# whabacivch/GC-SLAM

Measured on AMD Instinct MI355X. Metric: scans/sec (14-step pipeline) at 64k pts/scan, higher is better.
Workload: dtype f64

## Files before the change

gc-slam_amd/csrc/gcs_capi.cpp:

```cpp
#include "gcslam_hip.h"

#include <hip/hip_runtime.h>
#include <math.h>
#include <rccl/rccl.h>
#include <string.h>

#include <algorithm>
#include <atomic>
#include <sys/syscall.h>
#include <unistd.h>
#include <chrono>
#include <condition_variable>
#include <mutex>
#include <thread>
#include <string>
#include <vector>

#include "gcs_atlas.h"
#include "gcs_host.h"
#include "gcs_imu_odom_core.h"
#include "gcs_kernels.h"
#include "gcs_layout.h"
#include "gcs_live.h"
#include "gcs_math.h"
// ... 107 lines not shown
    int nblk;
    gcs_pmap* pm;
    int32_t n12, ncl;
    int32_t tiles12[GCS_LIVE_MAX_TILES], clear12[GCS_LIVE_MAX_TILES];
    int64_t tids12[GCS_LIVE_MAX_TILES];
    double ts12;
    int64_t seq12, next12;
    gcs_pmap_update_config ucfg;
    gcs_pmap_update_inputs uin;
  };
  PushJob push_jobs[2]{};
  int push_rc = 0;
  std::string push_err;
  uint64_t* h_gate = nullptr;
  uint64_t* d_gate = nullptr;
  double* d_gate_xi = nullptr;
  uint64_t gate_seq = 0, gate_next = 0;
  bool gate_on = false;
  bool gate_withhold = false;
  bool device_preint = false;
  bool device_imu_odom = false;
  bool io_dev_pending = false;
  hipStream_t io_stream = nullptr;
  double* h_io_stage = nullptr;
  double* d_io_win = nullptr;
  double* d_io_out = nullptr;
  double* h_io_out = nullptr;
  double* dh_io_out = nullptr;
  uint64_t* d_io_seq = nullptr;
  uint64_t io_seq = 0;
  int64_t io_rereads = 0, io_syncs = 0;
  hipEvent_t ev_preint = nullptr;
  bool ev_preint_pending = false;
  bool preint_pending = false;
  bool preint_host_pending = false;
  double* h_preint_in = nullptr;
  int64_t preint_in_cap = 0;
  double* h_preint_out = nullptr;
  int pts_blocks = 0;
  bool pts_fold_pending = false;
  double* d_scalars = nullptr;
  double* h_scalars = nullptr;
  double* d_scalars_mirror = nullptr;
  uint64_t mirror_seq = 0;
  int64_t mirror_scans = 0, mirror_rereads = 0, mirror_syncs = 0;
  int mirror_torn = 0;
  uint32_t h_err[4] = {0u, 0u, 0u, 0u};
  uint32_t* d_err = nullptr;
  uint32_t* d_members = nullptr;
  int capb = 32, capb_eff = 32;
  bool direct_buckets = true;
  bool sorted_sticky = false;
  bool use_direct = false;
  uint32_t spin_limit = 1u << 22;
  int inject_scan_fail = 0;
  bool legacy_points = [] {
    const char* e = getenv("GCSLAM_POINTS");
    return e && strcmp(e, "legacy") == 0;
  }();
  double* h_payload = nullptr;
  double* dh_payload = nullptr;
  double* d_payload = nullptr;
  double* d_payload_in = nullptr;
  int combine_delay_us = 0;
  int sendbuf_mode = -1;
  void* comm_seen = nullptr;
  int comm_world = 1;
  double* h_psum = nullptr;
  double* dh_psum = nullptr;
  hipStream_t comm_stream = nullptr;
  uint64_t pay_seq = 0;
  uint64_t* d_pay_seq = nullptr;
  int64_t pay_rereads = 0, pay_syncs = 0;
  Belief belief{};
  int map_mode = GCS_MAP_OWN;
  double map_rec[GCS_MAP_REC_LEN] = {};
  double lead_rec[GCS_MAP_REC_LEN] = {};
  bool have_lead_rec = false;
  bool prev_fac_valid = false;
  host::SpdFactor prev_fac;
  double prev_cov[DZ * DZ];
  double iw_nu[7], iw_Psi[7 * 36], Q[DZ * DZ];
  double last_dPsi[7 * 36], last_dnu[7];
  double meas_nu[3], meas_Psi[3 * 9], meas_cert[2] = {0.0, 0.0};
  double last_meas_dPsi[3 * 9], last_meas_dnu[3];
  bool have_last = false;
  int last_n_sel = 0, last_stride = 1;
  int budget_blocks = 0;
  double host_sums[10] = {};
  int64_t host_n[2] = {0, 0};
  static constexpr int kHostHist = 4096;
  std::vector<float> host_hist = std::vector<float>((size_t)kHostHist * 6, 0.0f);
  std::atomic<int64_t> worker_tid{0};
  bool budget_pending = false;
  bool self_budget = [] {
    const char* e = getenv("GCSLAM_SELF_BUDGET");
    return !(e && atoi(e) == 0);
  }();
  bool budget_self = false, recs_deferred = false;
  double2* d_mass_rows = nullptr;
  std::vector<double> wimu, wint;
  host::ImuOdomOut io;
  double grav[3] = {0.0, 0.0, 0.0};
  uint32_t timing_mask = 0;
  static constexpr int kEvRing = 256;
  std::vector<hipEvent_t> ev[kStages];
// ... 238 lines not shown
  a.t0 = t0;
  a.t1 = t1;
  memcpy(a.xi, xi, 6 * sizeof(double));
  memcpy(a.origin, c->cfg.lidar_origin, 3 * sizeof(double));
  a.tau = c->cfg.tau;
  a.bin_dirs = c->d_bin_dirs;
  a.n_bins = c->B;
  a.knn = c->d_knn;
  a.k = c->K;
  a.pools = c->d_pools;
  a.pool_bound = c->d_pool_bound;
  a.bin_ref = c->d_bin_ref;
  a.pool_width = c->pool_width;
  a.grid = c->G;
  a.recs = c->d_recs;
  a.keys = c->d_keys;
  a.slots = c->d_slots;
  a.counts = c->d_counts;
  if (c->use_direct) {
    a.members = c->d_members;
    a.capb = c->capb_eff;
    a.flags = c->d_flags;
    a.tile_shift = c->tile_shift;
    a.overflow = c->d_err + 2;
  }
  a.budget_partials = c->budget_self ? nullptr : c->d_partials;
  a.budget_blocks = c->budget_self ? 0 : c->budget_blocks;
  a.mass_rows = c->budget_self ? c->d_mass_rows : nullptr;
  c->recs_deferred = c->budget_self && c->cfg.mode == GCS_MODE_SCALE && !deskew_only;
  a.scalars = c->d_scalars;
  a.p0_out = p0_out;
  a.w_out = w_out;
  a.w_budget_out = wb_out;
  a.nearest_out = c->d_nearest;
  a.iz_out = iz_out;
  a.t_out = t_out;
  if (c->gate_next) {
    HIPCHK(c, launch_gate(c->d_gate, c->gate_next, c->d_gate_xi, c->d_err + 3, s));
    a.xi_dev = c->d_gate_xi;
    c->gate_next = 0;
  } else if (c->preint_pending) {
    a.xi_dev = c->d_gate_xi;
    c->preint_pending = false;
  }
  c->iz_valid = false;
  const bool scale = c->cfg.mode == GCS_MODE_SCALE && !deskew_only;
  if (deskew_only) {
    a.n_bins = 0;
    a.nearest_out = nullptr;
    a.members = nullptr;
  }
  c->pts_blocks = points_blocks(c->cap, scale);
  c->pts_fold_pending = scale && fold_later;
  MirrorArgs mir{};
  if (to_host && !c->pts_fold_pending) {
    mir.mirror = c->d_scalars_mirror;
    mir.err = c->d_err;
    mir.seq = ++c->mirror_seq;
    mir.torn = c->mirror_torn;
  }
  HIPCHK(c, launch_points(a, scale, c->d_part_pts, c->pts_blocks, !c->pts_fold_pending, s, ev.e0, ev.e1,
                          c->legacy_points, mir));
  return GCS_OK;
}

BinKernelArgs bin_args(gcs_ctx* c) {
  BinKernelArgs b{};
  b.recs = c->d_recs;
  b.perm = c->d_perm;
  if (c->use_direct) {
    b.members = c->d_members;
    b.capb = c->capb_eff;
  }
  b.starts = c->d_starts;
  b.counts = c->d_counts;
  b.flags = c->d_flags;
  b.tile_dirty = c->d_tile_dirty;
  b.tile_order = c->d_tile_order;
  b.tile_work = c->d_tile_work;
  b.rknn_off = c->d_rknn_off;
  b.rknn = c->d_rknn;
  b.rknn_local = c->d_rknn_local;
  b.tile_src_off = c->d_tile_src_off;
  b.tile_src = c->d_tile_src;
  b.bin_dirs = c->d_bin_dirs;
  b.map = c->d_map;
  b.n_bins = c->B;
  b.cap = c->cap;
  b.tile_bins = c->tile_bins;
  memcpy(b.origin, c->cfg.lidar_origin, 3 * sizeof(double));
  b.tau = c->cfg.tau;
  b.scan = c->d_scan;
  b.scalars = c->d_scalars;
  if (c->pts_fold_pending) {
    b.pts_partials = c->d_part_pts;
    b.pts_blocks = c->pts_blocks;
  }
  if (c->recs_deferred) {
    b.mass_rows = c->d_mass_rows;
    b.mass_nrows = c->pts_blocks;
  }
  if (c->d_counts) {
    b.zero_after = c->d_counts + c->B;
    b.n_zero_after = c->n_counts_words - c->B;
  }
  return b;
}

int stage_bins(gcs_ctx* c) {
  hipStream_t s = c->stream;
  BinKernelArgs b = bin_args(c);
  if (c->cfg.mode == GCS_MODE_SCALE) {
    if (!c->use_direct) {
      StageEv ev = stage_ev(c, ST_SORT);
      BucketArgs ba{};
      ba.n_bins = c->B;
      ba.k = c->K;
      ba.counts = c->d_counts;
      ba.keys = c->d_keys;
      ba.slots = c->d_slots;
      ba.knn = c->d_knn;
      ba.starts = c->d_starts;
      ba.scan_status = c->d_counts + c->B + 2;
      ba.scan_ticket = c->d_tickets;
      ba.slot_idx = c->d_sorted;
// ... 2599 lines not shown
```

gc-slam_amd/csrc/gcs_kernels.h:

```cpp
#pragma once
#include <hip/hip_runtime.h>
#include <stddef.h>
#include <stdint.h>

#include "gcs_layout.h"

namespace gcs {


struct ParseArgs {
  const uint8_t* data;
  int n, point_step;
  int off_x, off_y, off_z, off_ring, ring_datatype, off_t, t_datatype;
  double header_stamp;
  double R[9], tb[3];
  double* points;
  double* t;
  double* w;
  uint8_t* ring;
  uint32_t* ns_flag;
};

struct BudgetArgs {
  const double* w;
// ... 37 lines not shown
  int k;
  const int* pools;
  const float* pool_bound;
  const int* bin_ref;
  int pool_width, grid;
  PointRec* recs;
  uint32_t* keys;
  uint32_t* slots;
  uint32_t* counts;
  uint32_t* members;
  int capb;
  uint8_t* flags;
  int tile_shift;
  uint32_t* overflow;
  const double* budget_partials;
  int budget_blocks;
  double2* mass_rows;
  double* scalars;
  double* p0_out;
  double* w_out;
  double* w_budget_out;
  int* nearest_out;
  double* iz_out;
  double* t_out;
  const double* xi_dev;
};
constexpr uint64_t kGateTimeoutTicks = 20000000ull;

struct BucketArgs {
  int n_bins, k;
  const uint32_t* counts;
  const uint32_t* keys;
  const uint32_t* slots;
  const int* knn;
  uint32_t* starts;
  uint32_t* scan_status;
  uint32_t* scan_ticket;
  uint32_t* slot_idx;
  uint32_t* perm;
  uint8_t* flags;
  int tile_shift;
  uint32_t* err;
  uint32_t spin_limit;
  int inject_scan_fail;
};

struct BinKernelArgs {
  const PointRec* recs;
  const uint32_t* perm;
  const uint32_t* members;
  int capb;
  const uint32_t* starts;
  const uint32_t* counts;
  const uint8_t* flags;
  uint8_t* tile_dirty;
  const int* rknn_off;
  const int* rknn;
  const uint16_t* rknn_local;
  const int* tile_src_off;
  const int* tile_src;
  const double* bin_dirs;
  const double* map;
  int n_bins, cap;
  int tile_bins;
  double origin[3];
  double tau;
  double* scan;
  double* scalars;
  const double* pts_partials;
  int pts_blocks;
  const double2* mass_rows;
  int mass_nrows;
  uint32_t* zero_after;
  int n_zero_after;
  const int* tile_order;
  uint32_t* tile_work;
};

struct PushArgs {
  double R[9];
  double t[3];
  double Stt[9];
  double F[9];
  double G[9];
  double gamma;
};

hipError_t launch_parse(const ParseArgs& a, hipStream_t s);
hipError_t launch_budget(const BudgetArgs& a, int nblk, hipStream_t s, hipEvent_t e0, hipEvent_t e1);
int points_blocks(long cap, bool scale);
int points_max_blocks();
struct PreintArgs {
  const double* imu;
  int m;
  int n_tail;
  double tail_stamp;
  double t0, t1, sigma;
  double rotvec[3], gb[3], ab[3], g[3];
  int rotation_only;
  double* xi_dev;
  double* host_out;
};
hipError_t launch_preint(const PreintArgs& a, hipStream_t s);
constexpr int kImuOdomMaxM = 1024;
constexpr int kImuOdomStatWords = 24;
enum ImuOdomSmall : int {
  kIoPose0 = 0, kIoPosePred = 6, kIoMuPrev = 12, kIoMuInc = 34, kIoGravity = 56, kIoSigmaG = 59, kIoSigmaA = 68,
  kIoOdomPose = 77, kIoOdomCov = 83, kIoOdomTwist = 119, kIoOdomTwistCov = 125, kIoSmallLen = 161
};
struct ImuOdomDevArgs {
  const double* win;
  int m;
  double t_last_scan, t_scan, dt_sec;
  double planar_z_ref, planar_z_sigma, planar_vz_sigma;
  double* out;
  double* host;
  uint64_t* dseq;
};
hipError_t launch_imu_odom(const ImuOdomDevArgs& a, hipStream_t s);
hipError_t launch_gate(const uint64_t* gate, uint64_t seq, double* xi_out, uint32_t* err, hipStream_t s);
hipError_t launch_payload_out(const double* src, double* host, int n, uint64_t* dseq, hipStream_t s);
hipError_t launch_delay(int us, hipStream_t s);
hipError_t launch_points(const PointKernelArgs& a, bool scale, double* partials, int nblk, bool fold, hipStream_t s,
                         hipEvent_t e0, hipEvent_t e1, bool legacy = false, const MirrorArgs& mir = MirrorArgs{});
int scan_tiles(int n_bins);
hipError_t launch_bucketing(const BucketArgs& b, int n, hipStream_t s, hipEvent_t e0, hipEvent_t e1);
int bins_tile_for(long cap, int n_bins);
int bins_scale_blocks(int n_bins, int tile_bins);
int partial_stride(int nv);
size_t partials_need(long nblocks, int nv);
int bins_max_tile_sources(int tile_bins);
int bins_max_tile_entries(int tile_bins);
int bins_partial_nv();
int push_blocks(int n_bins);
hipError_t launch_bins_scale(const BinKernelArgs& a, double* partials, hipStream_t s, hipEvent_t e0, hipEvent_t e1,
                             hipEvent_t f0, hipEvent_t f1);
hipError_t launch_dense(const BinKernelArgs& a, double* bin_partials, double* partials, hipStream_t s, hipEvent_t e0,
                        hipEvent_t e1);
hipError_t launch_mf(const double* scan, const double* map, int B, double* partials, int nblk, double* scalars,
                     hipStream_t s, hipEvent_t e0, hipEvent_t e1);
hipError_t launch_pt(const double* scan, const double* map, const double* derived, int B, double* partials, int nblk,
                     double* scalars, const MirrorArgs& mir, const uint8_t* act, const uint8_t* touched,
                     hipStream_t s, hipEvent_t e0, hipEvent_t e1, PtClear clr = PtClear{});
hipError_t launch_tile_order(const uint8_t* active, const uint32_t* work, int n, int* order, hipStream_t s);
hipError_t launch_tile_order_variant(const uint8_t* active, const uint32_t* work, int n, int* order, bool xcd,
                                     hipStream_t s);
hipError_t launch_pushforward(const double* scan, double* map, double* derived, int B, const PushArgs& pa,
                              double* partials, double* scalars, const uint8_t* act, uint8_t* touched, hipStream_t s,
                              hipEvent_t e0, hipEvent_t e1);
hipError_t launch_map_derive(const double* map, double* derived, int B, double* partials, double* scalars,
                             uint8_t* touched, hipStream_t s);

}
```

gc-slam_amd/csrc/gcs_kernels.hip:

```cpp
#include <hip/hip_runtime.h>


#include "gcs_kernels.h"

#include <hip/hip_ext.h>
#include <string.h>
#include "gcs_layout.h"
#include "gcs_math.h"

namespace gcs {

constexpr int kBlock = 256;
constexpr int kWaves = kBlock / 64;

template <int NV>
__device__ __forceinline__ void wave_sum(double (&v)[NV]) {
#pragma unroll
  for (int off = 32; off >= 1; off >>= 1) {
#pragma unroll
    for (int k = 0; k < NV; ++k) v[k] += __shfl_xor(v[k], off, 64);
  }
}

template <int NV>
// ... 369 lines not shown
      for (int k = 0; k < 4; ++k) {
        v[0] += brow[k].x;
        v[1] += brow[k].y;
      }
      block_sum<2>(v, lds);
      if (threadIdx.x == 0) {
        s_mass[0] = v[0];
        s_mass[1] = v[0] / (v[1] + kEpsMass);
        if (blockIdx.x == 0) {
          a.scalars[SC_MASS_IN] = v[0];
          a.scalars[SC_MASS_SEL] = v[1];
          a.scalars[SC_MASS_SCALE] = s_mass[1];
        }
      }
      __syncthreads();
      mass_scale = s_mass[1];
      mass_in = s_mass[0];
    }
    if (!live) continue;
    const double wb = w_raw * mass_scale;
    const double wout = wb * win;
    if (a.t_out) a.t_out[i] = t;
    if constexpr (SCALE) {
      reinterpret_cast<double4*>(a.recs)[i] = make_double4(p0[0], p0[1], p0[2], wout * Z);
    } else if constexpr (KC != 0) {
      PointRec pr;
      pr.x = p0[0]; pr.y = p0[1]; pr.z = p0[2];
      pr.dx = d[0]; pr.dy = d[1]; pr.dz = d[2];
      pr.m = m; pr.wz = wout * Z;
      a.recs[i] = pr;
    }
    if (a.iz_out) a.iz_out[i] = Z;
    if (a.p0_out) { a.p0_out[3 * (size_t)i] = p0[0]; a.p0_out[3 * (size_t)i + 1] = p0[1]; a.p0_out[3 * (size_t)i + 2] = p0[2]; }
    if (a.w_out) a.w_out[i] = wout;
    if (a.w_budget_out) a.w_budget_out[i] = wb;
    if (a.nearest_out) a.nearest_out[i] = nearest;
    double wn = self ? wb : wb / (mass_in + kEpsMass);
    acc[0] += wb;
    acc[1] += wn * wn;
    acc[2] += wout;
    acc[3] += H;
    rmax = fmax(rmax, rm);
  }
  if (self) {
    block_sum<2>(msum, lds);
    if (threadIdx.x == 0) a.mass_rows[blockIdx.x] = make_double2(msum[0], msum[1]);
  }
  block_sum<4>(acc, lds);
  rmax = block_max(rmax, lds);
  double v[5] = {acc[0], acc[1], acc[2], acc[3], rmax};
  store_partials<5>(v, partials, blockIdx.x);
}

template <int KC>
__global__ __launch_bounds__(kBlock) __attribute__((amdgpu_waves_per_eu(4)))
void k_points_lean(PointKernelArgs a, double* partials) {
  constexpr int CG = KC < 8 ? KC : 8;
  constexpr int EG = 4;
  static_assert(KC % CG == 0, "candidate groups");
  __shared__ double lds[kWaves * 5];
  __shared__ double s_mass[2];
  const int nb = (int)gridDim.x;
  const int lb = (nb & 7) ? (int)blockIdx.x : (int)(blockIdx.x & 7u) * (nb >> 3) + (int)(blockIdx.x >> 3);
  static_assert(kBlock * 4 >= 1024, "k_budget launches at most 1024 blocks: four rows per thread");
  double2 brow[4];
#pragma unroll
  for (int k = 0; k < 4; ++k) {
    const int r = threadIdx.x + k * kBlock;
    brow[k] = r < a.budget_blocks ? *(const double2*)(a.budget_partials + (size_t)r * pstride<2>())
                                  : make_double2(0.0, 0.0);
  }
  const int i = lb * kBlock + (int)threadIdx.x;
  const bool live = i < a.cap;
  const bool valid = live && i < a.n_sel;
  double p[3] = {0.0, 0.0, 0.0}, t = 0.0, w_raw = 0.0;
  if (valid) {
    const size_t src = (size_t)i * (size_t)a.stride;
    if (a.xyz_f64) {
      const double* rec = (const double*)(a.xyz + src * (size_t)a.point_step);
      p[0] = rec[0]; p[1] = rec[1]; p[2] = rec[2];
    } else {
      const float* rec = (const float*)(a.xyz + src * (size_t)a.point_step);
      p[0] = (double)rec[0]; p[1] = (double)rec[1]; p[2] = (double)rec[2];
    }
    t = a.timestamps[src];
    w_raw = a.weights[src];
  }
  double bsum[2] = {0.0, 0.0};
  if (a.mass_rows) {
    if (valid) {
      const size_t src = (size_t)i * (size_t)a.stride;
      bsum[0] = w_raw;
      for (int q = 1; q < a.stride && src + q < (size_t)a.n_raw; ++q) bsum[0] += a.weights[src + q];
      bsum[1] = w_raw;
    }
  } else {
#pragma unroll
    for (int k = 0; k < 4; ++k) {
      bsum[0] += brow[k].x;
      bsum[1] += brow[k].y;
    }
  }
  double p0[3], d[3], win;
  {
    double xi[6];
#pragma unroll
    for (int k = 0; k < 6; ++k) xi[k] = a.xi_dev ? a.xi_dev[k] : a.xi[k];
    const double denom = a.t1 - a.t0 > 1e-12 ? a.t1 - a.t0 : 1e-12;
    const double alpha = (t - a.t0) / denom;
    deskew_point(alpha, xi, p, p0);
    win = smooth_window(t, a.t0, a.t1, kTimeWarpSigmaFrac * denom);
    ray_dir(p0[0], p0[1], p0[2], a.origin, d);
  }
  int nearest = 0;
  if (!(d[0] == 0.0 && d[1] == 0.0 && d[2] == 0.0)) {
    const size_t prow = (size_t)cube_cell(d[0], d[1], d[2], a.grid) * a.pool_width;
    const int4* pool = (const int4*)(a.pools + prow);
    const float* pbound = a.pool_bound + prow;
    const int nq = a.pool_width >> 2;
    double best = -INFINITY;
    for (int q = 0; q < nq; q += 2) {
      const int4 u0 = pool[q];
      const int4 u1 = q + 1 < nq ? pool[q + 1] : make_int4(-1, -1, -1, -1);
      const float bnext = q + 2 < nq ? pbound[4 * (q + 2)] : -2.0f;
      const int ids[8] = {u0.x, u0.y, u0.z, u0.w, u1.x, u1.y, u1.z, u1.w};
      double s[8];
#pragma unroll
      for (int u = 0; u < 8; ++u) {
        const double* bp = a.bin_dirs + 4 * (size_t)(ids[u] >= 0 ? ids[u] : 0);
        const double2 xy = *(const double2*)bp;
        const double sv = dot3_exact(d[0], d[1], d[2], xy.x, xy.y, bp[2]);
        s[u] = ids[u] >= 0 ? sv : -INFINITY;
      }
#pragma unroll
      for (int u = 0; u < 8; ++u) {
        if (s[u] > best) {
          best = s[u];
          nearest = ids[u];
        } else if (s[u] == best && ids[u] >= 0 && a.bin_ref[ids[u]] < a.bin_ref[nearest]) {
          nearest = ids[u];
        }
      }
      if (u1.w < 0 || (best > 0.0 && (double)bnext < best)) break;
    }
  }
  double e[KC];
  double m = -INFINITY;
  {
    const int* krow = a.knn + (size_t)nearest * KC;
#pragma unroll
    for (int k0 = 0; k0 < KC; k0 += CG) {
      int cid[CG];
#pragma unroll
      for (int k = 0; k < CG; k += 4) {
        const int4 c4 = *(const int4*)(krow + k0 + k);
        cid[k] = c4.x; cid[k + 1] = c4.y; cid[k + 2] = c4.z; cid[k + 3] = c4.w;
      }
      if (k0 > 0)
#pragma unroll
        for (int k = 0; k < CG; ++k) __asm__ volatile("" : "+v"(cid[k]) : "v"(m));
      double3 bd[CG];
#pragma unroll
      for (int k = 0; k < CG; ++k) {
        const double* bp = a.bin_dirs + 4 * (size_t)cid[k];
        const double2 xy = *(const double2*)bp;
        bd[k] = make_double3(xy.x, xy.y, bp[2]);
      }
#pragma unroll
      for (int k = 0; k < CG; ++k) {
        e[k0 + k] = dot3_exact(d[0], d[1], d[2], bd[k].x, bd[k].y, bd[k].z);
        m = fmax(m, e[k0 + k]);
      }
      if (CG < KC) __builtin_amdgcn_sched_barrier(0);
    }
  }
  const double inv_tau = 1.0 / a.tau;
  double Z = 0.0, sxe = 0.0;
#pragma unroll
  for (int k = 0; k < KC; ++k) {
    const double x = (e[k] - m) * inv_tau;
    e[k] = exp(x);
    Z += e[k];
    sxe += x * e[k];
    if ((k & (EG - 1)) == EG - 1) __builtin_amdgcn_sched_barrier(0);
  }
  const double iz = 1.0 / Z;
  double corr = 0.0, rm = 0.0;
#pragma unroll
  for (int k = 0; k < KC; ++k) {
    const double r = e[k] * iz;
    corr += r * __builtin_amdgcn_rcp(r + kEpsMass);
    rm = fmax(rm, r);
  }
  const double H = log(Z) - sxe * iz - kEpsMass * corr;
  if (valid) {
    const uint32_t sl = atomicAdd(a.counts + nearest, 1u);
    if (a.members) {
      if (sl < (uint32_t)a.capb) a.members[(size_t)nearest * a.capb + sl] = (uint32_t)i;
      else *a.overflow = 1u;
      if (sl == 0u) {
        const int ts = a.tile_shift;
        uint8_t* tf = a.flags + a.n_bins;
        const int* krow = a.knn + (size_t)nearest * KC;
        for (int k = 0; k < KC; k += 4) {
          const int4 c4 = *(const int4*)(krow + k);
          a.flags[c4.x] = 1; tf[c4.x >> ts] = 1;
          a.flags[c4.y] = 1; tf[c4.y >> ts] = 1;
          a.flags[c4.z] = 1; tf[c4.z >> ts] = 1;
          a.flags[c4.w] = 1; tf[c4.w >> ts] = 1;
        }
      }
    } else {
      a.slots[i] = sl;
    }
  }
  if (live && !a.members) a.keys[i] = valid ? (uint32_t)nearest : (uint32_t)a.n_bins;
  block_sum<2>(bsum, lds);
  if (threadIdx.x == 0) {
    if (a.mass_rows) {
      a.mass_rows[lb] = make_double2(bsum[0], bsum[1]);
      s_mass[0] = 0.0;
      s_mass[1] = 1.0;
    } else {
      s_mass[0] = bsum[0];
      s_mass[1] = bsum[0] / (bsum[1] + kEpsMass);
      if (lb == 0) {
        a.scalars[SC_MASS_IN] = bsum[0];
        a.scalars[SC_MASS_SEL] = bsum[1];
        a.scalars[SC_MASS_SCALE] = s_mass[1];
      }
    }
  }
  __syncthreads();
  const double mass_scale = s_mass[1], mass_in = s_mass[0];
  double acc[4] = {0.0, 0.0, 0.0, 0.0};
  double rmax = -INFINITY;
  if (live) {
    const double wb = w_raw * mass_scale;
    const double wout = wb * win;
    reinterpret_cast<double4*>(a.recs)[i] = make_double4(p0[0], p0[1], p0[2], wout * iz);
    if (a.t_out) a.t_out[i] = t;
    if (a.iz_out) a.iz_out[i] = iz;
    if (a.p0_out) { a.p0_out[3 * (size_t)i] = p0[0]; a.p0_out[3 * (size_t)i + 1] = p0[1]; a.p0_out[3 * (size_t)i + 2] = p0[2]; }
    if (a.w_out) a.w_out[i] = wout;
    if (a.w_budget_out) a.w_budget_out[i] = wb;
    if (a.nearest_out) a.nearest_out[i] = nearest;
    const double wn = a.mass_rows ? wb : wb / (mass_in + kEpsMass);
    acc[0] = 0.0 + wb;
    acc[1] = 0.0 + wn * wn;
    acc[2] = 0.0 + wout;
    acc[3] = 0.0 + H;
    rmax = fmax(rmax, rm);
  }
  block_sum<4>(acc, lds);
  rmax = block_max(rmax, lds);
  double v[5] = {acc[0], acc[1], acc[2], acc[3], rmax};
  store_partials<5>(v, partials, lb);
}

constexpr int kScanThreads = 256;
constexpr int kScanTile = 16 * kScanThreads;
constexpr int kLaneRank = 16;
constexpr int kRankMax = 8192;
constexpr uint32_t kLbAgg = 1u << 30, kLbPre = 2u << 30, kLbVal = (1u << 30) - 1u;

__global__ __launch_bounds__(kScanThreads) void k_scan(const uint32_t* __restrict__ counts, int n, uint32_t* status,
                                                       uint32_t* ticket, uint32_t* start, uint32_t* err,
                                                       uint32_t spin_limit, int inject_fail) {
  constexpr int kSW = kScanThreads / 64;
  __shared__ uint32_t wsum[kSW];
  __shared__ uint32_t s_tile, s_excl;
  const int t = threadIdx.x, lane = t & 63, wid = t >> 6;
  if (t == 0) s_tile = atomicAdd(ticket, 1u);
  __syncthreads();
  const uint32_t tile = s_tile;
  const int base = (int)tile * kScanTile + 16 * t;
  uint32_t v[16];
  if (base + 16 <= n) {
#pragma unroll
    for (int q = 0; q < 4; ++q) {
      const uint4 u = *(const uint4*)(counts + base + 4 * q);
      v[4 * q] = u.x; v[4 * q + 1] = u.y; v[4 * q + 2] = u.z; v[4 * q + 3] = u.w;
    }
  } else {
#pragma unroll
    for (int j = 0; j < 16; ++j) v[j] = (base + j < n) ? counts[base + j] : 0u;
  }
  uint32_t tot = 0;
#pragma unroll
  for (int j = 0; j < 16; ++j) tot += v[j];
  uint32_t x = tot;
  for (int off = 1; off < 64; off <<= 1) {
    uint32_t y = __shfl_up(x, off, 64);
    if (lane >= off) x += y;
  }
  if (lane == 63) wsum[wid] = x;
  __syncthreads();
  if (wid == 0) {
    uint32_t agg = 0;
    for (int w = 0; w < kSW; ++w) agg += wsum[w];
    uint32_t excl = 0;
    if (tile == 0) {
      if (lane == 0) __hip_atomic_store(status, kLbPre | agg, __ATOMIC_RELAXED, __HIP_MEMORY_SCOPE_AGENT);
    } else {
      if (lane == 0) __hip_atomic_store(status + tile, kLbAgg | agg, __ATOMIC_RELAXED, __HIP_MEMORY_SCOPE_AGENT);
      uint32_t spins = 0;
      bool failed = inject_fail && tile == 1;
      int w0 = failed ? -1 : (int)tile - 1;
      while (w0 >= 0) {
        const int j = w0 - lane;
// ... 426 lines not shown
      if (lane == 0) s_mw[wid] = ws;
      __syncthreads();
      if (t == 0) {
        double m_in, m_sel;
        const double msc = mass_scale_of<NW>(s_mw, &m_in, &m_sel);
        a.scalars[SC_MASS_IN] = m_in;
        a.scalars[SC_MASS_SEL] = m_sel;
        a.scalars[SC_MASS_SCALE] = msc;
        const double q = msc / (m_in + kEpsMass);
        pv[0] *= msc;
        pv[1] = pv[1] * q * q;
        pv[2] *= msc;
      }
      __syncthreads();
    }
    if (t == 0 && a.pts_partials)
      for (int f = 0; f < 5; ++f) a.scalars[SC_DESKEW_WIN + f] = pv[f];
  }
  const bool tile_active = a.flags[a.n_bins + tile] != 0;
  const bool tile_dirty = a.tile_dirty[tile] != 0;
  const int q_t = t < nb ? a.rknn_off[b0 + t] : 0;
  const int q0 = a.rknn_off[b0], q1t = a.rknn_off[b0 + nb];
  const int s0 = a.tile_src_off[tile];
  const int ns = a.tile_src_off[tile + 1] - s0;
  if (!tile_active && !tile_dirty) {
    PROF(6);
    PROFV(7, 2);
    return;
  }
  if (t == 0 && tile_active && !tile_dirty) a.tile_dirty[tile] = 1;
  if (!tile_active) {
    __syncthreads();
    if (t == 0) a.tile_dirty[tile] = 0;
    if (DALL || t < TB) {
      double z[19], c5[5] = {0.0, 0.0, 0.0, 0.0, -INFINITY};
#pragma unroll
      for (int f = 0; f < 19; ++f) z[f] = 0.0;
      if (t < nb) finalize_bin(z, a.scan, a.n_bins, b0 + t, c5);
      if (t == 0) {
        double v[kBinNV];
#pragma unroll
        for (int f = 0; f < kBinNV; ++f) v[f] = 0.0;
        v[3] = (double)nb * c5[3];
        v[4] = c5[4];
        store_partials<kBinNV>(v, partials, tile);
      }
    }
    PROF(6);
    PROFV(7, 0);
    return;
  }
  const int own_b = DALL ? t / LANES : t;
  const bool own = DALL ? (t % LANES == 0 && own_b < nb) : t < nb;
  const bool act_t = t < nb && a.flags[b0 + t];
  const bool own_act = DALL ? own && a.flags[b0 + own_b] : act_t;
  MapDir mapv{0.0, 0.0, 0.0, 0.0};
  if (own_act) mapv = load_map_dir(a.map, a.n_bins, b0 + own_b);
  if (t < nb) s_bd[t] = *(const double4*)(a.bin_dirs + 4 * (size_t)(b0 + t));
  if (t < 3) s_org[t] = a.origin[t];
  if (t < nb) s_q[t] = q_t;
  if (t == 0) s_q[nb] = q1t;
  if (t < TB) s_act[t] = act_t ? 1 : 0;
  {
    constexpr int RL = (kMaxRl + NT - 1) / NT, SR = (kMaxSrc + NT - 1) / NT;
    double2 mw[4];
#pragma unroll
    for (int k = 0; k < 4; ++k) {
      const int r = t + k * NT;
      const bool ok = a.mass_rows && r < a.mass_nrows;
      mw[k] = ok ? a.mass_rows[r] : make_double2(0.0, 0.0);
    }
    uint16_t rl[RL];
#pragma unroll
    for (int k = 0; k < RL; ++k) {
      const int q = q0 + t + k * NT;
      rl[k] = q < q1t ? a.rknn_local[q] : (uint16_t)0;
    }
    int src[SR];
#pragma unroll
    for (int k = 0; k < SR; ++k) src[k] = t + k * NT < ns ? a.tile_src[s0 + t + k * NT] : 0;
    uint32_t cn[SR], st[SR];
#pragma unroll
    for (int k = 0; k < SR; ++k) {
      cn[k] = t + k * NT < ns ? a.counts[src[k]] : 0u;
      if (a.members) cn[k] = min(cn[k], (uint32_t)a.capb);
      st[k] = t + k * NT < ns ? (a.members ? (uint32_t)src[k] * (uint32_t)a.capb : a.starts[src[k]]) : 0u;
    }
#pragma unroll
    for (int k = 0; k < RL; ++k)
      if (q0 + t + k * NT < q1t) s_rl[t + k * NT] = rl[k];
#pragma unroll
    for (int k = 0; k < SR; ++k)
      if (t + k * NT < ns) {
        s_cnt[t + k * NT] = cn[k];
        s_st[t + k * NT] = st[k];
      }
    if (a.mass_rows) {
      const double2 ws = mass_rows_wave_pre<NT>(a.mass_rows, a.mass_nrows, mw);
      if (lane == 0) s_mw[wid] = ws;
    }
  }
  __syncthreads();
  PROF(1);
  if (a.mass_rows && t == 0) s_msc = mass_scale_of<NW>(s_mw);
  {
    const int rb = t / LANES, rq = t % LANES;
    int qa = 0, lo = 0, hi = 0;
    if (s_act[rb]) {
      qa = s_q[rb] - q0;
      const int n = s_q[rb + 1] - q0 - qa;
      lo = qa + n * rq / LANES;
      hi = qa + n * (rq + 1) / LANES;
    }
    uint32_t w = 0;
    int nz = 0;
    for (int q = lo; q < hi; q += 4) {
      uint16_t j[4];
#pragma unroll
      for (int u = 0; u < 4; ++u) j[u] = q + u < hi ? s_rl[q + u] : (uint16_t)0;
#pragma unroll
      for (int u = 0; u < 4; ++u) {
        const uint32_t c = q + u < hi ? s_cnt[j[u]] : 0u;
        w += c;
        nz += c ? 1 : 0;
      }
    }
    int x = nz;
#pragma unroll
    for (int off = 1; off < LANES; off <<= 1) {
      const int y = __shfl_up(x, off, 64);
      if (rq >= off) x += y;
    }
    int e = qa + (x - nz);
    for (int q = lo; q < hi; q += 4) {
      uint16_t j[4];
#pragma unroll
      for (int u = 0; u < 4; ++u) j[u] = q + u < hi ? s_rl[q + u] : (uint16_t)0;
#pragma unroll
      for (int u = 0; u < 4; ++u)
        if (q + u < hi && s_cnt[j[u]]) s_rlc[e++] = j[u];
    }
#pragma unroll
    for (int off = 1; off < LANES; off <<= 1) w += (uint32_t)__shfl_xor((int)w, off, 64);
    if (rq == 0) s_work[rb] = w;
  }
  const int chunk = (ns + NT - 1) / NT;
  const int j0 = min(ns, t * chunk), j1 = min(ns, j0 + chunk);
  uint32_t mine = 0;
  for (int j = j0; j < j1; ++j) mine += s_cnt[j];
  uint32_t x = mine;
  for (int off = 1; off < 64; off <<= 1) {
    uint32_t y = __shfl_up(x, off, 64);
    if (lane >= off) x += y;
  }
  if (lane == 63) s_wsum[wid] = x;
  __syncthreads();
  uint32_t run = x - mine;
  for (int w = 0; w < wid; ++w) run += s_wsum[w];
  for (int j = j0; j < j1; ++j) {
    s_off[j] = run;
    run += s_cnt[j];
  }
  uint32_t total = 0;
#pragma unroll
  for (int w = 0; w < NW; ++w) total += s_wsum[w];
  const bool staged = total <= (uint32_t)STAGE;
  if (t == 0 && a.tile_work) a.tile_work[tile] = total;
  PROFV(8, total);
#ifdef GCS_PHASE_PROF
  if (t == 0) {
    uint32_t mx = 0, sm = 0;
    for (int i = 0; i < TB; ++i) { mx = max(mx, s_work[i]); sm += s_work[i]; }
    g_prof[blockIdx.x * 16 + 9] = mx;
    g_prof[blockIdx.x * 16 + 10] = sm;
  }
#endif
  __syncthreads();
  PROF(2);
  if (staged) {
    constexpr int RPT = (STAGE + NT - 1) / NT;
    uint32_t pi[RPT], dst[RPT], sid[RPT];
#pragma unroll
    for (int k = 0; k < RPT; ++k) {
      const uint32_t r = t + k * NT;
      pi[k] = 0u;
      dst[k] = r;
      sid[k] = 0u;
      if (r < total) {
        int lo = 0, hi = ns - 1;
        while (lo < hi) {
          int mid = (lo + hi + 1) >> 1;
          if (s_off[mid] <= r) lo = mid; else hi = mid - 1;
        }
        sid[k] = (uint32_t)a.tile_src[s0 + lo];
        const uint32_t pos = s_st[lo] + (r - s_off[lo]);
        if (a.members) {
          const uint32_t c = s_cnt[lo];
          const uint4* row = (const uint4*)(a.members + s_st[lo]);
          const uint32_t me = a.members[pos];
          uint32_t rank = 0;
          for (uint32_t q = 0; q < c; q += 4) {
            const uint4 m4 = row[q >> 2];
            rank += (m4.x < me) + (q + 1 < c && m4.y < me) + (q + 2 < c && m4.z < me) + (q + 3 < c && m4.w < me);
          }
          pi[k] = me;
          dst[k] = s_off[lo] + rank;
        } else {
          pi[k] = a.perm[pos];
        }
// ... 888 lines not shown
  }
  __asm__ volatile("" ::: "memory");
  for (int k = 0; k < 6; ++k)
    xi_out[k] = open ? __longlong_as_double((long long)__hip_atomic_load(gate + 1 + k, __ATOMIC_RELAXED,
                                                                        __HIP_MEMORY_SCOPE_SYSTEM))
                     : 0.0;
  if (!open) *err = 1u;
}

__global__ __launch_bounds__(kBlock) void k_payload_out(const double* __restrict__ src, double* host, int n,
                                                        uint64_t* dseq) {
  __shared__ unsigned long long lh[kWaves];
  unsigned long long h = 0;
  uint64_t* hw = reinterpret_cast<uint64_t*>(host);
  for (int i = threadIdx.x; i < n; i += kBlock) {
    const uint64_t w = (uint64_t)__double_as_longlong(src[i]);
    hw[i] = w;
    h += mirror_word_hash(w, (uint32_t)i);
  }
#pragma unroll
  for (int off = 32; off >= 1; off >>= 1) h += __shfl_xor(h, off, 64);
  if ((threadIdx.x & 63) == 0) lh[threadIdx.x >> 6] = h;
  __threadfence_system();
  __syncthreads();
  if (threadIdx.x == 0) {
    const uint64_t seq = *dseq + 1u;
    *dseq = seq;
    uint64_t sum = mirror_word_hash(seq, (uint32_t)n);
    for (int k = 0; k < kWaves; ++k) sum += lh[k];
    hw[n + 1] = sum;
    hw[n] = seq;
  }
}
hipError_t launch_payload_out(const double* src, double* host, int n, uint64_t* dseq, hipStream_t s) {
  hipLaunchKernelGGL(k_payload_out, dim3(1), dim3(kBlock), 0, s, src, host, n, dseq);
  return hipGetLastError();
}

__global__ __launch_bounds__(64) void k_delay(uint32_t us) {
  const uint64_t t0 = wall_clock64();
  while (wall_clock64() - t0 < 100ull * (uint64_t)us) __builtin_amdgcn_s_sleep(64);
}

hipError_t launch_delay(int us, hipStream_t s) {
  hipLaunchKernelGGL(k_delay, dim3(1), dim3(64), 0, s, (uint32_t)us);
  return hipGetLastError();
}

hipError_t launch_gate(const uint64_t* gate, uint64_t seq, double* xi_out, uint32_t* err, hipStream_t s) {
  hipLaunchKernelGGL(k_gate, dim3(1), dim3(64), 0, s, gate, seq, xi_out, err);
  return hipGetLastError();
}

constexpr int kPointsMaxBlocks = 4096;
int points_max_blocks() { return kPointsMaxBlocks; }
int points_blocks(long cap, bool scale) {
  const long need = (cap + kBlock - 1) / kBlock;
  return (int)std::max(1L, std::min((long)(scale ? kPointsMaxBlocks : 1024), need));
}

hipError_t launch_points(const PointKernelArgs& a, bool scale, double* partials, int nblk, bool fold, hipStream_t s,
                         hipEvent_t e0, hipEvent_t e1, bool legacy, const MirrorArgs& mir) {
  hipEvent_t ek = fold ? nullptr : e1;
  if (scale && !legacy && (long)nblk * kBlock >= (long)a.cap) {
    switch (a.k) {
      case 8: hipExtLaunchKernelGGL(k_points_lean<8>, dim3(nblk), dim3(kBlock), 0, s, e0, ek, 0, a, partials); break;
      case 16: hipExtLaunchKernelGGL(k_points_lean<16>, dim3(nblk), dim3(kBlock), 0, s, e0, ek, 0, a, partials); break;
      case 32: hipExtLaunchKernelGGL(k_points_lean<32>, dim3(nblk), dim3(kBlock), 0, s, e0, ek, 0, a, partials); break;
      default: return hipErrorInvalidValue;
    }
  } else if (scale) {
    switch (a.k) {
      case 8: hipExtLaunchKernelGGL((k_points<true, 8>), dim3(nblk), dim3(kBlock), 0, s, e0, ek, 0, a, partials); break;
      case 16: hipExtLaunchKernelGGL((k_points<true, 16>), dim3(nblk), dim3(kBlock), 0, s, e0, ek, 0, a, partials); break;
      case 32: hipExtLaunchKernelGGL((k_points<true, 32>), dim3(nblk), dim3(kBlock), 0, s, e0, ek, 0, a, partials); break;
      default: return hipErrorInvalidValue;
    }
  } else if (a.n_bins == 0) {
    hipExtLaunchKernelGGL((k_points<false, 0>), dim3(nblk), dim3(kBlock), 0, s, e0, ek, 0, a, partials);
  } else {
    hipExtLaunchKernelGGL((k_points<false, 1>), dim3(nblk), dim3(kBlock), 0, s, e0, ek, 0, a, partials);
  }
  if (fold) GCS_FINAL_M(5, 16u, FIN_POINTS, nblk, s, e1, partials, a.scalars, mir);
  return hipGetLastError();
}

int scan_tiles(int n_bins) { return (n_bins + kScanTile - 1) / kScanTile; }

hipError_t launch_bucketing(const BucketArgs& b, int n, hipStream_t s, hipEvent_t e0, hipEvent_t e1) {
  hipExtLaunchKernelGGL(k_scan, dim3(scan_tiles(b.n_bins)), dim3(kScanThreads), 0, s, e0, nullptr, 0,
                        (const uint32_t*)b.counts, b.n_bins, b.scan_status, b.scan_ticket, b.starts, b.err,
                        b.spin_limit, b.inject_scan_fail);
  hipLaunchKernelGGL(k_place, dim3(grid_for(n, 2048)), dim3(kBlock), 0, s, (const uint32_t*)b.keys,
                     (const uint32_t*)b.slots, (const uint32_t*)b.starts, n, b.n_bins, b.slot_idx);
  hipExtLaunchKernelGGL(k_bucket_rank, dim3((b.n_bins + kBlock - 1) / kBlock), dim3(kBlock), 0, s, nullptr, e1, 0, b,
                        n);
  return hipGetLastError();
}

int bins_tile_for(long cap, int n_bins) {
  if (const char* e = getenv("GCSLAM_BIN_TILE")) {
    const int v = atoi(e);
    if (v == 32 || v == 64 || v == 128 || v == 256) return v;
  }
  return (long)cap * 5 < (long)n_bins * 2 ? 128 : 64;
}
int bins_scale_blocks(int n_bins, int tile_bins) { return (n_bins + tile_bins - 1) / tile_bins; }
int bins_partial_nv() { return kBinNV; }

hipError_t launch_bins_scale(const BinKernelArgs& a, double* partials, hipStream_t s, hipEvent_t e0, hipEvent_t e1,
                             hipEvent_t f0, hipEvent_t f1) {
  const int nblk = bins_scale_blocks(a.n_bins, a.tile_bins);
  const bool big = (long)a.cap * 5 >= (long)a.n_bins * 2;
  if (a.tile_bins == 32)
    hipExtLaunchKernelGGL((k_bins_scale<kStageSmall, 32, 8, false>), dim3(nblk), dim3(256), 0, s, e0, e1, 0, a, partials);
  else if (a.tile_bins == 128 && big)
    hipExtLaunchKernelGGL((k_bins_scale<kStage128Big, 128, 2, false>), dim3(nblk), dim3(256), 0, s, e0, e1, 0, a, partials);
// ... 61 lines not shown
```

Baseline: 8908.

## Derive bin flags in bin kernel and merge lean points-kernel reductions

The lean points kernel no longer scatters per-bin activity flags for every kNN candidate. It writes only deduplicated tile flags, and the bin kernel now rebuilds the per-bin flags from its own work counts when derive_flags is set. The points kernel also merges the mass-row reduction and the accumulator reduction into a single wave/LDS pass, which removes a block-wide sum and a barrier. It moves the counts atomic earlier so its latency overlaps the softmax math, and adds optional phase-profiling timestamps. The aim is to cut scattered byte writes and synchronization in the points stage, at the cost of slightly more logic in the bin kernel.

```diff
diff --git a/gc-slam_amd/csrc/gcs_capi.cpp b/gc-slam_amd/csrc/gcs_capi.cpp
--- a/gc-slam_amd/csrc/gcs_capi.cpp
+++ b/gc-slam_amd/csrc/gcs_capi.cpp
@@ -183,6 +183,7 @@
   bool direct_buckets = true;
   bool sorted_sticky = false;
   bool use_direct = false;
+  bool pts_lean = false;
   uint32_t spin_limit = 1u << 22;
   int inject_scan_fail = 0;
   bool legacy_points = [] {
@@ -527,6 +528,7 @@
   }
   c->pts_blocks = points_blocks(c->cap, scale);
   c->pts_fold_pending = scale && fold_later;
+  c->pts_lean = scale && points_lean_for(c->cap, c->pts_blocks, c->legacy_points);
   MirrorArgs mir{};
   if (to_host && !c->pts_fold_pending) {
     mir.mirror = c->d_scalars_mirror;
@@ -546,6 +548,7 @@
   if (c->use_direct) {
     b.members = c->d_members;
     b.capb = c->capb_eff;
+    b.derive_flags = c->pts_lean ? 1 : 0;
   }
   b.starts = c->d_starts;
   b.counts = c->d_counts;
diff --git a/gc-slam_amd/csrc/gcs_kernels.h b/gc-slam_amd/csrc/gcs_kernels.h
--- a/gc-slam_amd/csrc/gcs_kernels.h
+++ b/gc-slam_amd/csrc/gcs_kernels.h
@@ -113,7 +113,8 @@
   int capb;
   const uint32_t* starts;
   const uint32_t* counts;
-  const uint8_t* flags;
+  uint8_t* flags;
+  int derive_flags;
   uint8_t* tile_dirty;
   const int* rknn_off;
   const int* rknn;
@@ -184,6 +185,7 @@
 hipError_t launch_delay(int us, hipStream_t s);
 hipError_t launch_points(const PointKernelArgs& a, bool scale, double* partials, int nblk, bool fold, hipStream_t s,
                          hipEvent_t e0, hipEvent_t e1, bool legacy = false, const MirrorArgs& mir = MirrorArgs{});
+bool points_lean_for(long cap, int nblk, bool legacy);
 int scan_tiles(int n_bins);
 hipError_t launch_bucketing(const BucketArgs& b, int n, hipStream_t s, hipEvent_t e0, hipEvent_t e1);
 int bins_tile_for(long cap, int n_bins);
diff --git a/gc-slam_amd/csrc/gcs_kernels.hip b/gc-slam_amd/csrc/gcs_kernels.hip
--- a/gc-slam_amd/csrc/gcs_kernels.hip
+++ b/gc-slam_amd/csrc/gcs_kernels.hip
@@ -445,17 +445,36 @@
   store_partials<5>(v, partials, blockIdx.x);
 }
 
+constexpr int kPointsMaxBlocks = 4096;
+
+#ifdef GCS_PHASE_PROF
+__device__ unsigned long long g_prof_pts[kPointsMaxBlocks * 8];
+extern "C" int gcs_debug_prof_points(unsigned long long* out, int n) {
+  return (int)hipMemcpyFromSymbol(out, HIP_SYMBOL(g_prof_pts), (size_t)n * sizeof(unsigned long long));
+}
+#define PPROF(k)                                                          \
+  do {                                                                    \
+    __builtin_amdgcn_sched_barrier(0);                                    \
+    __builtin_amdgcn_s_waitcnt(0);                                        \
+    if (threadIdx.x == 0) g_prof_pts[lb * 8 + (k)] = wall_clock64();      \
+    __builtin_amdgcn_sched_barrier(0);                                    \
+  } while (0)
+#else
+#define PPROF(k)
+#endif
+
 template <int KC>
 __global__ __launch_bounds__(kBlock) __attribute__((amdgpu_waves_per_eu(4)))
 void k_points_lean(PointKernelArgs a, double* partials) {
   constexpr int CG = KC < 8 ? KC : 8;
   constexpr int EG = 4;
   static_assert(KC % CG == 0, "candidate groups");
-  __shared__ double lds[kWaves * 5];
+  __shared__ double lds[kWaves * 7];
   __shared__ double s_mass[2];
   const int nb = (int)gridDim.x;
   const int lb = (nb & 7) ? (int)blockIdx.x : (int)(blockIdx.x & 7u) * (nb >> 3) + (int)(blockIdx.x >> 3);
   static_assert(kBlock * 4 >= 1024, "k_budget launches at most 1024 blocks: four rows per thread");
+  PPROF(0);
   double2 brow[4];
 #pragma unroll
   for (int k = 0; k < 4; ++k) {
@@ -494,6 +513,7 @@
       bsum[1] += brow[k].y;
     }
   }
+  PPROF(1);
   double p0[3], d[3], win;
   {
     double xi[6];
@@ -505,6 +525,7 @@
     win = smooth_window(t, a.t0, a.t1, kTimeWarpSigmaFrac * denom);
     ray_dir(p0[0], p0[1], p0[2], a.origin, d);
   }
+  PPROF(2);
   int nearest = 0;
   if (!(d[0] == 0.0 && d[1] == 0.0 && d[2] == 0.0)) {
     const size_t prow = (size_t)cube_cell(d[0], d[1], d[2], a.grid) * a.pool_width;
@@ -537,8 +558,10 @@
       if (u1.w < 0 || (best > 0.0 && (double)bnext < best)) break;
     }
   }
+  PPROF(3);
   double e[KC];
   double m = -INFINITY;
+  int ctile[KC];
   {
     const int* krow = a.knn + (size_t)nearest * KC;
 #pragma unroll
@@ -564,9 +587,14 @@
         e[k0 + k] = dot3_exact(d[0], d[1], d[2], bd[k].x, bd[k].y, bd[k].z);
         m = fmax(m, e[k0 + k]);
       }
+#pragma unroll
+      for (int k = 0; k < CG; ++k) ctile[k0 + k] = cid[k] >> a.tile_shift;
       if (CG < KC) __builtin_amdgcn_sched_barrier(0);
     }
   }
+  PPROF(4);
+  uint32_t sl = 0u;
+  if (valid) sl = atomicAdd(a.counts + nearest, 1u);
   const double inv_tau = 1.0 / a.tau;
   double Z = 0.0, sxe = 0.0;
 #pragma unroll
@@ -586,35 +614,11 @@
     rm = fmax(rm, r);
   }
   const double H = log(Z) - sxe * iz - kEpsMass * corr;
-  if (valid) {
-    const uint32_t sl = atomicAdd(a.counts + nearest, 1u);
-    if (a.members) {
-      if (sl < (uint32_t)a.capb) a.members[(size_t)nearest * a.capb + sl] = (uint32_t)i;
-      else *a.overflow = 1u;
-      if (sl == 0u) {
-        const int ts = a.tile_shift;
-        uint8_t* tf = a.flags + a.n_bins;
-        const int* krow = a.knn + (size_t)nearest * KC;
-        for (int k = 0; k < KC; k += 4) {
-          const int4 c4 = *(const int4*)(krow + k);
-          a.flags[c4.x] = 1; tf[c4.x >> ts] = 1;
-          a.flags[c4.y] = 1; tf[c4.y >> ts] = 1;
-          a.flags[c4.z] = 1; tf[c4.z >> ts] = 1;
-          a.flags[c4.w] = 1; tf[c4.w >> ts] = 1;
-        }
-      }
-    } else {
-      a.slots[i] = sl;
-    }
-  }
-  if (live && !a.members) a.keys[i] = valid ? (uint32_t)nearest : (uint32_t)a.n_bins;
-  block_sum<2>(bsum, lds);
-  if (threadIdx.x == 0) {
-    if (a.mass_rows) {
-      a.mass_rows[lb] = make_double2(bsum[0], bsum[1]);
-      s_mass[0] = 0.0;
-      s_mass[1] = 1.0;
-    } else {
+  PPROF(5);
+  double mass_scale = 1.0, mass_in = 0.0;
+  if (!a.mass_rows) {
+    block_sum<2>(bsum, lds);
+    if (threadIdx.x == 0) {
       s_mass[0] = bsum[0];
       s_mass[1] = bsum[0] / (bsum[1] + kEpsMass);
       if (lb == 0) {
@@ -623,14 +627,55 @@
         a.scalars[SC_MASS_SCALE] = s_mass[1];
       }
     }
-  }
-  __syncthreads();
-  const double mass_scale = s_mass[1], mass_in = s_mass[0];
+    __syncthreads();
+    mass_scale = s_mass[1];
+    mass_in = s_mass[0];
+  }
+  const double wb = w_raw * mass_scale;
+  const double wout = wb * win;
   double acc[4] = {0.0, 0.0, 0.0, 0.0};
   double rmax = -INFINITY;
   if (live) {
-    const double wb = w_raw * mass_scale;
-    const double wout = wb * win;
+    const double wn = a.mass_rows ? wb : wb / (mass_in + kEpsMass);
+    acc[0] = 0.0 + wb;
+    acc[1] = 0.0 + wn * wn;
+    acc[2] = 0.0 + wout;
+    acc[3] = 0.0 + H;
+    rmax = fmax(rmax, rm);
+  }
+  double row[5], mrow[2] = {0.0, 0.0};
+  if (a.mass_rows) {
+    double s6[6] = {bsum[0], bsum[1], acc[0], acc[1], acc[2], acc[3]};
+    wave_sum<6>(s6);
+    rmax = wave_max(rmax);
+    const int lane = threadIdx.x & 63, wid = threadIdx.x >> 6;
+    if (lane == 0) {
+#pragma unroll
+      for (int k = 0; k < 6; ++k) lds[wid * 7 + k] = s6[k];
+      lds[wid * 7 + 6] = rmax;
+    }
+    __syncthreads();
+    if (threadIdx.x == 0) {
+      double r[7];
+#pragma unroll
+      for (int k = 0; k < 7; ++k) {
+        double x = lds[k];
+        for (int w = 1; w < kWaves; ++w) x = k == 6 ? fmax(x, lds[w * 7 + k]) : x + lds[w * 7 + k];
+        r[k] = x;
+      }
+      mrow[0] = r[0]; mrow[1] = r[1];
+#pragma unroll
+      for (int k = 0; k < 5; ++k) row[k] = r[2 + k];
+    }
+  } else {
+    block_sum<4>(acc, lds);
+    rmax = block_max(rmax, lds);
+#pragma unroll
+    for (int k = 0; k < 4; ++k) row[k] = acc[k];
+    row[4] = rmax;
+  }
+  PPROF(6);
+  if (live) {
     reinterpret_cast<double4*>(a.recs)[i] = make_double4(p0[0], p0[1], p0[2], wout * iz);
     if (a.t_out) a.t_out[i] = t;
     if (a.iz_out) a.iz_out[i] = iz;
@@ -638,17 +683,25 @@
     if (a.w_out) a.w_out[i] = wout;
     if (a.w_budget_out) a.w_budget_out[i] = wb;
     if (a.nearest_out) a.nearest_out[i] = nearest;
-    const double wn = a.mass_rows ? wb : wb / (mass_in + kEpsMass);
-    acc[0] = 0.0 + wb;
-    acc[1] = 0.0 + wn * wn;
-    acc[2] = 0.0 + wout;
-    acc[3] = 0.0 + H;
-    rmax = fmax(rmax, rm);
-  }
-  block_sum<4>(acc, lds);
-  rmax = block_max(rmax, lds);
-  double v[5] = {acc[0], acc[1], acc[2], acc[3], rmax};
-  store_partials<5>(v, partials, lb);
+    if (!a.members) a.keys[i] = valid ? (uint32_t)nearest : (uint32_t)a.n_bins;
+  }
+  if (valid) {
+    if (a.members) {
+      if (sl < (uint32_t)a.capb) a.members[(size_t)nearest * a.capb + sl] = (uint32_t)i;
+      else *a.overflow = 1u;
+      if (sl == 0u) {
+        uint8_t* const tf = a.flags + a.n_bins;
+#pragma unroll
+        for (int k = 0; k < KC; ++k)
+          if (k == 0 || ctile[k] != ctile[k - 1]) tf[ctile[k]] = 1;
+      }
+    } else {
+      a.slots[i] = sl;
+    }
+  }
+  if (a.mass_rows && threadIdx.x == 0) a.mass_rows[lb] = make_double2(mrow[0], mrow[1]);
+  store_partials<5>(row, partials, lb);
+  PPROF(7);
 }
 
 constexpr int kScanThreads = 256;
@@ -1181,8 +1234,9 @@
   }
   const int own_b = DALL ? t / LANES : t;
   const bool own = DALL ? (t % LANES == 0 && own_b < nb) : t < nb;
-  const bool act_t = t < nb && a.flags[b0 + t];
-  const bool own_act = DALL ? own && a.flags[b0 + own_b] : act_t;
+  const bool derive = a.derive_flags != 0;
+  const bool act_t = t < nb && (derive || a.flags[b0 + t]);
+  bool own_act = DALL ? own && (derive || a.flags[b0 + own_b]) : act_t;
   MapDir mapv{0.0, 0.0, 0.0, 0.0};
   if (own_act) mapv = load_map_dir(a.map, a.n_bins, b0 + own_b);
   if (t < nb) s_bd[t] = *(const double4*)(a.bin_dirs + 4 * (size_t)(b0 + t));
@@ -1284,6 +1338,10 @@
   }
   if (lane == 63) s_wsum[wid] = x;
   __syncthreads();
+  if (derive) {
+    if (t < nb) a.flags[b0 + t] = s_work[t] != 0u ? 1 : 0;
+    own_act = own && s_work[own_b] != 0u;
+  }
   uint32_t run = x - mine;
   for (int w = 0; w < wid; ++w) run += s_wsum[w];
   for (int j = j0; j < j1; ++j) {
@@ -2278,17 +2336,18 @@
   return hipGetLastError();
 }
 
-constexpr int kPointsMaxBlocks = 4096;
 int points_max_blocks() { return kPointsMaxBlocks; }
 int points_blocks(long cap, bool scale) {
   const long need = (cap + kBlock - 1) / kBlock;
   return (int)std::max(1L, std::min((long)(scale ? kPointsMaxBlocks : 1024), need));
 }
 
+bool points_lean_for(long cap, int nblk, bool legacy) { return !legacy && (long)nblk * kBlock >= cap; }
+
 hipError_t launch_points(const PointKernelArgs& a, bool scale, double* partials, int nblk, bool fold, hipStream_t s,
                          hipEvent_t e0, hipEvent_t e1, bool legacy, const MirrorArgs& mir) {
   hipEvent_t ek = fold ? nullptr : e1;
-  if (scale && !legacy && (long)nblk * kBlock >= (long)a.cap) {
+  if (scale && points_lean_for(a.cap, nblk, legacy)) {
     switch (a.k) {
       case 8: hipExtLaunchKernelGGL(k_points_lean<8>, dim3(nblk), dim3(kBlock), 0, s, e0, ek, 0, a, partials); break;
       case 16: hipExtLaunchKernelGGL(k_points_lean<16>, dim3(nblk), dim3(kBlock), 0, s, e0, ek, 0, a, partials); break;
```

Measured after the change: 8648. -2.9%, worse.
